# yizhiwang96/Slice3D

Measured on AMD Instinct MI355X. Metric: occupancy query-points/sec (U-Net encode + per-query decode, 256^2 x 12 slices), higher is better.
Workload: dtype f16x3

## Files before the change

include/slice3d_hip.h:

```cpp
#ifndef SLICE3D_HIP_H
#define SLICE3D_HIP_H

#include <stddef.h>
#include <stdint.h>

#ifdef __cplusplus
extern "C" {
#endif

#define S3D_VERSION 118
#define S3D_E_ARG (-1)
#define S3D_E_WORKSPACE (-2)

#define S3D_N_LEVELS 5
#define S3D_D_MODEL 128
#define S3D_N_LAYERS 3
#define S3D_FFN 2048
#define S3D_N_TOKENS_MAX 13

#define S3D_PREC_F32 0
#define S3D_PREC_F16X3 1
#define S3D_PREC_F16 2
#define S3D_PREC_BF16 3

int s3d_version(void);
const char* s3d_last_error(void);


typedef struct {
    const float* w;
    const float* b;
    const float* bn[4];
} S3dConvParams;

typedef struct {
    S3dConvParams enc[13];
    S3dConvParams trans_c;
    S3dConvParams trans_up[4];
    S3dConvParams up_t[4];
    S3dConvParams up_c1[4];
    S3dConvParams up_c2[4];
    S3dConvParams outc;
    const float* emds;
    int n_slices;
} S3dUNetParams;

size_t s3d_unet_packed_bytes(int n_slices);
int s3d_unet_pack(const S3dUNetParams* params_host, void* packed, size_t packed_bytes, void* stream);

typedef struct {
    float* level[S3D_N_LEVELS];
    int n_img;
    int size;
} S3dPyramid;

size_t s3d_unet_workspace_bytes(int batch, int size, int n_slices);
int s3d_unet_encode_fwd(const void* packed, const float* img, const S3dPyramid* out,
                        float* slices_rec, int batch, int size, int n_slices, int prec,
                        void* workspace, size_t workspace_bytes, void* stream);

typedef struct {
    const float* in_proj_w;  const float* in_proj_b;
    const float* out_proj_w; const float* out_proj_b;
// ... 49 lines not shown
    const float* std;
} S3dVggParams;
size_t s3d_vgg_packed_bytes(void);
int s3d_vgg_pack(const S3dVggParams* params_host, void* packed, size_t packed_bytes, void* stream);
size_t s3d_vgg_workspace_bytes(int n_img, int size);
int s3d_vgg_loss_fwd(const void* packed, const float* pred, const float* target, int n_img, int size,
                     float* loss_out, void* workspace, size_t workspace_bytes, void* stream);

typedef struct {
    S3dConvParams conv[13];
} S3dVgg16BnParams;
typedef struct {
    float* level[5];
    int n_img;
    int size;
} S3dGtPyramid;
size_t s3d_gt_encoder_packed_bytes(void);
int s3d_gt_encoder_pack(const S3dVgg16BnParams* params_host, void* packed, size_t packed_bytes, void* stream);
size_t s3d_gt_encoder_workspace_bytes(int n_img, int size);
int s3d_gt_encode_fwd(const void* packed, const float* img_slices, const S3dGtPyramid* out, int n_img, int size,
                      int prec, void* workspace, size_t workspace_bytes, void* stream);

typedef struct {
    const float* pts_w[3];  const float* pts_b[3];
    const float* local_w[2]; const float* local_b[2];
    S3dLayerParams layer[S3D_N_LAYERS];
    const float* fc_out_w; const float* fc_out_b;
} S3dGtHeadParams;
size_t s3d_gt_head_packed_bytes(void);
int s3d_gt_head_pack(const S3dGtHeadParams* params_host, void* packed, size_t packed_bytes, void* stream);
typedef struct {
    float* proj[4];
    const float* fine;
    int n_img;
    int size;
} S3dGtLatent;
int s3d_gt_latent_build(const void* head_packed, const S3dGtPyramid* pyr, const S3dGtLatent* out, int prec,
                        void* stream);
size_t s3d_gt_decode_workspace_bytes(int batch, long n_qry, int n_slices);
int s3d_gt_decode_points_fwd(const void* head_packed, const S3dGtLatent* latent, const float* qry,
                             const float* rot, const float* trans, int flip_yz, float* sdf_out, int batch,
                             long n_qry, int n_slices, int prec, void* workspace, size_t workspace_bytes,
                             void* stream);
int s3d_gt_decode_grid_fwd(const void* head_packed, const S3dGtLatent* latent, const float* trans, int nx,
                           float box, float* logits_out, int n_slices, int prec, void* workspace,
                           size_t workspace_bytes, void* stream);

size_t s3d_conv_packed_bytes(int cout, int cin0, int cin1, int ks);
int s3d_conv_pack(const float* w, const float* bias, int cout, int cin0, int cin1, int ks, void* packed,
                  size_t packed_bytes, void* stream);
int s3d_conv_fwd(const void* packed, const float* x0, const float* x1, const float* residual, float* out, int N,
                 int H, int W, int cout, int cin0, int cin1, int ks, int prec, void* workspace,
                 size_t workspace_bytes, void* stream);
size_t s3d_group_norm_stats_floats(int N, int groups);
int s3d_conv_gn_supported(int cout, int cin0, int cin1, int ks, int prec, int H, int W, int has_workspace);
typedef struct {
    const float* part;
    int nsplit;
    const void* conv_packed;
    int cout, cin0, cin1, ks;
    const float* residual;
    float* out;
} S3dConvPartial;
int s3d_group_norm_table_fwd(const float* x0, int c0, const float* x1, int c1, const float* gamma, const float* beta,
                             const float* film, long film_stride, float* table, float* stats, int N, int HW, int groups,
                             float eps, const S3dConvPartial* x0_partial, void* stream);
int s3d_group_norm_partial_fwd(const S3dConvPartial* x0_partial, const float* gamma, const float* beta, const float* film,
                               long film_stride, float* y, float* stats, int N, int HW, int groups, float eps, int silu,
                               void* stream);
int s3d_conv_gn_fwd(const void* packed, const float* x0, const float* x1, const float* residual, float* out, int N, int H,
                    int W, int cout, int cin0, int cin1, int ks, int prec, const float* table, int silu, void* workspace,
                    size_t workspace_bytes, int* nsplit_out, void* stream);
int s3d_conv_finish_fwd(const S3dConvPartial* partial, int N, int H, int W, void* stream);
int s3d_group_norm_fwd(const float* x, const float* gamma, const float* beta, const float* film, float* y,
                       float* stats, int N, int HW, int C, int groups, float eps, int silu, void* stream);
int s3d_group_norm_film_fwd(const float* x, const float* gamma, const float* beta, const float* film, long film_stride,
                            float* y, float* stats, int N, int HW, int C, int groups, float eps, int silu, void* stream);
int s3d_group_norm2_fwd(const float* x0, int c0, const float* x1, int c1, const float* gamma, const float* beta,
                        const float* film, float* y, float* stats, int N, int HW, int groups, float eps, int silu,
                        void* stream);
int s3d_qkv_attention_fwd(const float* qkv, float* out, int N, int T, int heads, int ch, int prec, void* stream);
size_t s3d_qkv_attention_ws_bytes(int N, int T, int heads, int ch);
int s3d_qkv_attention_ws_fwd(const float* qkv, float* out, int N, int T, int heads, int ch, void* ws, size_t ws_bytes,
                             void* stream);
int s3d_resample2x_fwd(const float* x, float* y, int N, int H, int W, int C, int up, void* stream);
int s3d_small_linear_fwd(const float* x, const float* w, const float* b, float* out, int N, int K, int M,
                         int silu_in, void* stream);
int s3d_timestep_embedding_fwd(const float* t, float* out, int N, int dim, float max_period, void* stream);
int s3d_add_fwd(const float* a, const float* b, float* out, long n, void* stream);
int s3d_nchw_to_nhwc_pad(const float* in, float* out, int n, int c, int h, int w, int cpad, void* stream);
int s3d_add_nchw_fwd(const float* a, const float* b, float* out, int n, int c, int h, int w, void* stream);

int s3d_conv_strided_fwd(const void* packed, const float* x, float* out, int N, int Hin, int Win, int Hout, int Wout, int cout,
                         int cin, int ks, int stride, int pad_origin, int prec, void* stream);
int s3d_wide_attention_fwd(const float* qkv, float* out, int N, int T, int C, int prec, void* stream);
int s3d_image_normalize_fwd(const float* x, const float* mean, const float* std, float* y, int n, int c, int h, int w,
                            void* stream);

typedef int (*s3d_all_reduce_sum_fn)(void* user, float* device_buf, long n_floats, void* stream);
typedef struct {
    s3d_all_reduce_sum_fn all_reduce_sum;
    void* user;
    int world_size;
    float* scratch;
} S3dSyncBn;
typedef struct {
// ... 121 lines not shown
```

slice3d_amd/_lib.py:

```python
import ctypes as C
import os

_HERE = os.path.dirname(os.path.abspath(__file__))
LIB_PATH = os.environ.get("S3D_HIP_LIB") or os.path.join(_HERE, "csrc", "libslice3d_hip.so")

N_LEVELS = 5
N_LAYERS = 3
PREC_F32 = 0
PREC_F16X3 = 1
PREC_F16 = 2
PREC_BF16 = 3
PREC = {"f32": PREC_F32, "f16x3": PREC_F16X3, "f16": PREC_F16, "bf16": PREC_BF16}
PROF_UNET, PROF_LATENT, PROF_SAMPLE, PROF_ATTN, PROF_FFN, PROF_FFN_FINAL, PROF_VGG, PROF_SAMPLE_PYR = range(8)
PROF_NAMES = ("unet_encode", "latent_build", "sample_tokens", "attn_layer", "ffn_layer", "ffn_final", "vgg_loss",
              "sample_pyramid")

c_float_p = C.POINTER(C.c_float)


class S3dConvParams(C.Structure):
    _fields_ = [("w", C.c_void_p), ("b", C.c_void_p), ("bn", C.c_void_p * 4)]


class S3dUNetParams(C.Structure):
# ... 51 lines not shown

class S3dGtHeadParams(C.Structure):
    _fields_ = [("pts_w", C.c_void_p * 3), ("pts_b", C.c_void_p * 3), ("local_w", C.c_void_p * 2),
                ("local_b", C.c_void_p * 2), ("layer", S3dLayerParams * N_LAYERS),
                ("fc_out_w", C.c_void_p), ("fc_out_b", C.c_void_p)]


class S3dGtLatent(C.Structure):
    _fields_ = [("proj", C.c_void_p * 4), ("fine", C.c_void_p), ("n_img", C.c_int), ("size", C.c_int)]


class S3dLatent(C.Structure):
    _fields_ = [("proj", C.c_void_p * 3), ("fine", C.c_void_p * 2), ("n_img", C.c_int),
                ("size", C.c_int)]


_vp, _i, _l, _sz, _f = C.c_void_p, C.c_int, C.c_long, C.c_size_t, C.c_float
SYMBOLS = {
    "s3d_version": (_i, []),
    "s3d_last_error": (C.c_char_p, []),
    "s3d_unet_packed_bytes": (_sz, [_i]),
    "s3d_unet_pack": (_i, [C.POINTER(S3dUNetParams), _vp, _sz, _vp]),
    "s3d_unet_workspace_bytes": (_sz, [_i, _i, _i]),
    "s3d_unet_encode_fwd": (_i, [_vp, _vp, C.POINTER(S3dPyramid), _vp, _i, _i, _i, _i, _vp, _sz, _vp]),
    "s3d_head_packed_bytes": (_sz, []),
    "s3d_head_pack": (_i, [C.POINTER(S3dHeadParams), _vp, _sz, _vp]),
    "s3d_latent_build": (_i, [_vp, C.POINTER(S3dPyramid), C.POINTER(S3dLatent), _i, _vp]),
    "s3d_decode_workspace_bytes": (_sz, [_i, _l, _i]),
    "s3d_decode_workspace_bytes_min": (_sz, [_i, _l, _i]),
    "s3d_decode_set_lanes": (_i, [_i]),
    "s3d_decode_set_last_fused": (_i, [_i]),
    "s3d_decode_set_shared_footprint": (_i, [_i]),
    "s3d_decode_points_fwd": (_i, [_vp, C.POINTER(S3dLatent), _vp, _vp, _vp, _i, _vp, _i, _l, _i, _i,
                                   _vp, _sz, _vp]),
    "s3d_decode_stages_floats": (_sz, [_i, _l, _i]),
    "s3d_decode_points_stages_fwd": (_i, [_vp, C.POINTER(S3dLatent), _vp, _vp, _vp, _i, _vp, _vp, _i, _l, _i, _i,
                                          _vp, _sz, _vp]),
    "s3d_decode_grid_fwd": (_i, [_vp, C.POINTER(S3dLatent), _vp, _i, _f, _vp, _i, _i, _vp, _sz, _vp]),
    "s3d_decode_grid_slab_fwd": (_i, [_vp, C.POINTER(S3dLatent), _vp, _i, _f, _l, _l, _vp, _i, _i, _vp, _sz, _vp]),
    "s3d_gt_encoder_packed_bytes": (_sz, []),
    "s3d_gt_encoder_pack": (_i, [C.POINTER(S3dVgg16BnParams), _vp, _sz, _vp]),
    "s3d_gt_encoder_workspace_bytes": (_sz, [_i, _i]),
    "s3d_gt_encode_fwd": (_i, [_vp, _vp, C.POINTER(S3dGtPyramid), _i, _i, _i, _vp, _sz, _vp]),
    "s3d_gt_head_packed_bytes": (_sz, []),
    "s3d_gt_head_pack": (_i, [C.POINTER(S3dGtHeadParams), _vp, _sz, _vp]),
    "s3d_gt_latent_build": (_i, [_vp, C.POINTER(S3dGtPyramid), C.POINTER(S3dGtLatent), _i, _vp]),
    "s3d_gt_decode_workspace_bytes": (_sz, [_i, _l, _i]),
    "s3d_gt_decode_points_fwd": (_i, [_vp, C.POINTER(S3dGtLatent), _vp, _vp, _vp, _i, _vp, _i, _l, _i, _i,
                                      _vp, _sz, _vp]),
    "s3d_gt_decode_grid_fwd": (_i, [_vp, C.POINTER(S3dGtLatent), _vp, _i, _f, _vp, _i, _i, _vp, _sz, _vp]),
    "s3d_conv_packed_bytes": (_sz, [_i, _i, _i, _i]),
    "s3d_conv_pack": (_i, [_vp, _vp, _i, _i, _i, _i, _vp, _sz, _vp]),
    "s3d_conv_fwd": (_i, [_vp, _vp, _vp, _vp, _vp, _i, _i, _i, _i, _i, _i, _i, _i, _vp, _sz, _vp]),
    "s3d_group_norm_stats_floats": (_sz, [_i, _i]),
    "s3d_group_norm_table_fwd": (_i, [_vp, _i, _vp, _i, _vp, _vp, _vp, C.c_long, _vp, _vp, _i, _i, _i, _f, _vp, _vp]),
    "s3d_group_norm_partial_fwd": (_i, [_vp, _vp, _vp, _vp, C.c_long, _vp, _vp, _i, _i, _i, _f, _i, _vp]),
    "s3d_conv_gn_supported": (_i, [_i, _i, _i, _i, _i, _i, _i, _i]),
    "s3d_conv_gn_fwd": (_i, [_vp, _vp, _vp, _vp, _vp, _i, _i, _i, _i, _i, _i, _i, _i, _vp, _i, _vp, _sz, _vp, _vp]),
    "s3d_conv_finish_fwd": (_i, [_vp, _i, _i, _i, _vp]),
    "s3d_group_norm_fwd": (_i, [_vp, _vp, _vp, _vp, _vp, _vp, _i, _i, _i, _i, _f, _i, _vp]),
    "s3d_group_norm_film_fwd": (_i, [_vp, _vp, _vp, _vp, C.c_long, _vp, _vp, _i, _i, _i, _i, _f, _i, _vp]),
    "s3d_group_norm2_fwd": (_i, [_vp, _i, _vp, _i, _vp, _vp, _vp, _vp, _vp, _i, _i, _i, _f, _i, _vp]),
    "s3d_qkv_attention_fwd": (_i, [_vp, _vp, _i, _i, _i, _i, _i, _vp]),
    "s3d_qkv_attention_ws_bytes": (_sz, [_i, _i, _i, _i]),
    "s3d_qkv_attention_ws_fwd": (_i, [_vp, _vp, _i, _i, _i, _i, _vp, _sz, _vp]),
    "s3d_resample2x_fwd": (_i, [_vp, _vp, _i, _i, _i, _i, _i, _vp]),
    "s3d_small_linear_fwd": (_i, [_vp, _vp, _vp, _vp, _i, _i, _i, _i, _vp]),
    "s3d_timestep_embedding_fwd": (_i, [_vp, _vp, _i, _i, _f, _vp]),
    "s3d_add_fwd": (_i, [_vp, _vp, _vp, _l, _vp]),
    "s3d_nchw_to_nhwc_pad": (_i, [_vp, _vp, _i, _i, _i, _i, _i, _vp]),
    "s3d_add_nchw_fwd": (_i, [_vp, _vp, _vp, _i, _i, _i, _i, _vp]),
    "s3d_conv_strided_fwd": (_i, [_vp, _vp, _vp, _i, _i, _i, _i, _i, _i, _i, _i, _i, _i, _i, _vp]),
    "s3d_wide_attention_fwd": (_i, [_vp, _vp, _i, _i, _i, _i, _vp]),
    "s3d_image_normalize_fwd": (_i, [_vp, _vp, _vp, _vp, _i, _i, _i, _i, _vp]),
    "s3d_vgg_packed_bytes": (_sz, []),
    "s3d_vgg_pack": (_i, [C.POINTER(S3dVggParams), _vp, _sz, _vp]),
    "s3d_vgg_workspace_bytes": (_sz, [_i, _i]),
    "s3d_vgg_loss_fwd": (_i, [_vp, _vp, _vp, _i, _i, _vp, _vp, _sz, _vp]),
    "s3d_train_workspace_bytes": (_sz, [_i, _i, _l, _i]),
    "s3d_train_fwd_bwd": (_i, [C.POINTER(S3dUNetParams), C.POINTER(S3dHeadParams), C.POINTER(S3dVggParams),
                               C.POINTER(S3dUNetParams), C.POINTER(S3dHeadParams), C.POINTER(S3dTrainBatch),
                               _i, _i, _l, _i, _f, C.c_ulonglong, _i, _vp, _vp, _vp, _vp, _sz, _vp]),
    "s3d_train_fwd": (_i, [C.POINTER(S3dUNetParams), C.POINTER(S3dHeadParams), C.POINTER(S3dVggParams),
                           C.POINTER(S3dTrainBatch), _i, _i, _l, _i, _f, C.c_ulonglong, _i, _vp, _vp, _vp, _vp, _sz, _vp]),
    "s3d_train_bwd": (_i, [C.POINTER(S3dUNetParams), C.POINTER(S3dHeadParams), C.POINTER(S3dVggParams),
                           C.POINTER(S3dUNetParams), C.POINTER(S3dHeadParams), C.POINTER(S3dTrainBatch),
                           _i, _i, _l, _i, _f, C.c_ulonglong, _i, _vp, _vp, _f, _f, _vp, _vp, _sz, _vp]),
    "s3d_gt_train_workspace_bytes": (_sz, [_i, _i, _l, _i]),
    "s3d_gt_train_fwd_bwd": (_i, [C.POINTER(S3dVgg16BnParams), C.POINTER(S3dGtHeadParams),
                                  C.POINTER(S3dVgg16BnParams), C.POINTER(S3dGtHeadParams), C.POINTER(S3dTrainBatch),
                                  _i, _i, _l, _i, _f, C.c_ulonglong, _i, _vp, _vp, _vp, _sz, _vp]),
    "s3d_dropout_mask": (_i, [C.c_ulonglong, _i, C.c_ulonglong, _l, _f, _vp, _vp]),
    "s3d_adam_step": (_i, [_vp, _vp, _vp, _vp, _l, _f, _f, _f, _f, _i, _vp]),
    "s3d_adam_step_multi": (_i, [_vp, _vp, _vp, _i, _vp, _vp, _vp, _f, _f, _f, _f, _i, _vp]),
    "s3d_prof_enable": (_i, [_i]),
    "s3d_range_push": (_i, [C.c_char_p]),
    "s3d_range_pop": (_i, []),
    "s3d_prof_read": (_i, [_i, C.POINTER(C.c_double), C.POINTER(C.c_long)]),
    "s3d_project_coord_fwd": (_i, [_vp, _vp, _vp, _i, _l, _vp]),
    "s3d_query_sort_workspace_bytes": (_sz, [_i, _l]),
    "s3d_query_sort": (_i, [_vp, _vp, _vp, _i, _i, _l, _vp, _vp, _sz, _vp]),
    "s3d_sample_pyramid_workspace_bytes": (_sz, [_i, _l]),
    "s3d_sample_pyramid_fwd": (_i, [C.POINTER(S3dPyramid), _vp, _vp, _i, _i, _l, _vp, _sz, _vp]),
    "s3d_sample_planes_fwd": (_i, [_vp, _vp, _vp, _i, _i, _i, _i, _l, _vp]),
    "s3d_mise_dev_workspace_bytes": (_sz, [_i, _i]),
    "s3d_mise_dev_create": (_vp, [_vp, _sz, _i, _i, C.c_double, _vp]),
# ... 81 lines not shown
```

slice3d_amd/csrc/api.hip:

```cpp
#include <dlfcn.h>
#include <stdarg.h>
#include <string.h>

#include <vector>
#include <mutex>

#include <math.h>

#include "conv.h"
#include "decode.h"
#include "train.h"
#include "ldm_ops.h"

static thread_local char g_err[512] = "";

void s3d_set_error(const char* fmt, ...) {
    va_list ap;
    va_start(ap, fmt);
    vsnprintf(g_err, sizeof(g_err), fmt, ap);
    va_end(ap);
}

extern "C" int s3d_version(void) { return S3D_VERSION; }
extern "C" const char* s3d_last_error(void) { return g_err; }
// ... 220 lines not shown
        return S3D_E_WORKSPACE;
    }
    float* base = (float*)packed;
    TRY(pack_encoder(P->enc, base, L.E, st));
    if (hipMemcpyAsync(base + L.enc0_raw, P->enc[0].w, 64 * 27 * sizeof(float), hipMemcpyDeviceToDevice, st) != hipSuccess) {
        s3d_set_error("unet_pack: copy of conv1_1's weight failed");
        return S3D_E_ARG;
    }
    TRY(pack_linear(P->trans_c.w, base + L.trans_c.w, 512, 512, 640, 640, 0, st));
    TRY(pack_linear(P->trans_c.w, base + L.trans_c.w16, 512, 512, 640, 640, 0, st, 1));
    TRY(launch_fold_bn(P->trans_c.b, nullptr, base + L.trans_c.scale, base + L.trans_c.shift, 512, 512, 1, 0, st));
    for (int i = 0; i < 4; ++i) {
        const int C = kUpC[i], Ct = C / 2;
        TRY(pack_linear(P->trans_up[i].w, base + L.trans_up[i].w, Ct, Ct, C, C, 0, st));
        TRY(pack_linear(P->trans_up[i].w, base + L.trans_up[i].w16, Ct, Ct, C, C, 0, st, 1));
        TRY(launch_fold_bn(P->trans_up[i].b, nullptr, base + L.trans_up[i].scale, base + L.trans_up[i].shift, Ct,
                           Ct, 1, 0, st));
        {
            PackArgs a = {};
            a.src = P->up_t[i].w; a.dst = base + L.up_t[i].w; a.kind = S3D_PACK_CONVT;
            a.n_valid = 4 * Ct; a.n_pad = 4 * Ct; a.KU_total = C / 16; a.u_off = 0; a.ku_seg = C / 16;
            a.k_valid = C; a.ct = Ct;
            TRY(launch_pack(a, st));
            a.f16 = 1; a.dst = base + L.up_t[i].w16;
            TRY(launch_pack(a, st));
            TRY(launch_fold_bn(P->up_t[i].b, nullptr, base + L.up_t[i].scale, base + L.up_t[i].shift, Ct, 4 * Ct, 4,
                               0, st));
        }
        TRY(pack_conv3(P->up_c1[i].w, base + L.up_c1[i].w, Ct, Ct, C, 0, Ct, L.up_c1[i].KU, 0, 9, st));
        TRY(pack_conv3(P->up_c1[i].w, base + L.up_c1[i].w, Ct, Ct, C, Ct, Ct, L.up_c1[i].KU, 9 * Ct / 16, 9, st));
        TRY(pack_conv3(P->up_c1[i].w, base + L.up_c1[i].w16, Ct, Ct, C, 0, Ct, L.up_c1[i].KU, 0, 9, st, 1));
        TRY(pack_conv3(P->up_c1[i].w, base + L.up_c1[i].w16, Ct, Ct, C, Ct, Ct, L.up_c1[i].KU, 9 * Ct / 16, 9, st, 1));
        TRY(launch_fold_bn(nullptr, P->up_c1[i].bn, base + L.up_c1[i].scale, base + L.up_c1[i].shift, Ct, Ct, 1, 0,
                           st));
        TRY(pack_conv3(P->up_c2[i].w, base + L.up_c2[i].w, Ct, Ct, Ct, 0, Ct, L.up_c2[i].KU, 0, 9, st));
        TRY(pack_conv3(P->up_c2[i].w, base + L.up_c2[i].w16, Ct, Ct, Ct, 0, Ct, L.up_c2[i].KU, 0, 9, st, 1));
        TRY(launch_fold_bn(nullptr, P->up_c2[i].bn, base + L.up_c2[i].scale, base + L.up_c2[i].shift, Ct, Ct, 1, 0,
                           st));
    }
    TRY(pack_linear(P->outc.w, base + L.outc.w, 3, 16, 32, 32, 0, st));
    TRY(pack_linear(P->outc.w, base + L.outc.w16, 3, 16, 32, 32, 0, st, 1));
    TRY(launch_fold_bn(P->outc.b, nullptr, base + L.outc.scale, base + L.outc.shift, 3, 16, 1, 0, st));
    hipError_t e = hipMemcpyAsync(base + L.emds, P->emds, (size_t)P->n_slices * 128 * sizeof(float),
                                  hipMemcpyDeviceToDevice, st);
    if (e != hipSuccess) {
        s3d_set_error("unet_pack: memcpy failed: %s", hipGetErrorString(e));
        return (int)e;
    }
    return 0;
}

#define S3D_SPLITK_FLOATS ((size_t)4718592)
struct UNetWs {
    size_t in16, a, b, x[5], p[4], proj, up, mid, splitk;
    size_t total;
};
static UNetWs unet_ws(int B, int S, int ns) {
    UNetWs W;
    size_t off = 0;
    auto take = [&](size_t n) {
        size_t o = off;
        off += (n + 63) / 64 * 64;
        return o;
    };
    const size_t px = (size_t)B * S * S;
    W.in16 = take(px * 16);
    W.a = take(px * 64);
    W.b = take(px * 64 / 2);
    const int xc[5] = {64, 128, 256, 512, 512};
    for (int i = 0; i < 5; ++i) W.x[i] = take((px >> (2 * i)) * xc[i]);
    for (int i = 0; i < 4; ++i) W.p[i] = take((px >> (2 * (i + 1))) * xc[i]);
    W.proj = take(px * 32);
    W.up = take(px * ns * 32);
    W.mid = take(px * ns * 32);
    W.splitk = take(S3D_SPLITK_FLOATS);
    W.total = off;
    return W;
}

extern "C" size_t s3d_unet_workspace_bytes(int batch, int size, int n_slices) {
    return unet_ws(batch, size, n_slices).total * sizeof(float);
}

static ConvLaunch conv_desc(const float* base, const PackedConv& pc, int prec, int N, int H, int W, int ks, int act) {
    ConvLaunch c = {};
    c.wpk16 = prec != S3D_PREC_F32 ? (const void*)(base + pc.w16) : nullptr;
    c.single_pass = prec == S3D_PREC_F16;
    c.N = N; c.H = H; c.W = W; c.ks = ks;
    c.CoutPad = pc.cout_pad; c.wpk = base + pc.w; c.KU = pc.KU;
    c.scale = base + pc.scale; c.shift = base + pc.shift;
    c.act = act; c.out_mode = S3D_OUT_NHWC; c.cout_store = pc.cout_pad; c.out_cstride = pc.cout_pad;
    return c;
}
static ConvSrc plain_src(const float* p, int C) { return ConvSrc{p, C, 1, 0, 0}; }

static ConvLaunch proj_desc(const float* w, const void* w16, bool single, int n, int k, const float* x, int N, int H,
                            int W, float* out, const float* shift = nullptr, int act = S3D_ACT_NONE) {
    ConvLaunch c = {};
    c.N = N; c.H = H; c.W = W; c.ks = 1;
    c.CoutPad = n; c.wpk = w; c.KU = k / 16;
    c.wpk16 = w16; c.single_pass = single;
    c.shift = shift; c.act = act;
    c.out_mode = S3D_OUT_NHWC; c.cout_store = n; c.out_cstride = n;
    c.nsrc = 1;
    c.src[0] = plain_src(x, k);
    c.out = out;
    return c;
}

static int encoder_fwd(const float* base, const EncLayout& E, int prec, int N, int S, int first, const float* in,
                       float* const tap[5], float* const pp[2], float* const pool[4], float* splitk, hipStream_t st) {
    const float* cur = in;
    int curC = first ? kEncCout[0] : 16, res = S, tap_i = 0, flip = first;
    for (int i = first; i < 13; ++i) {
        ConvLaunch c = conv_desc(base, E.enc[i], prec, N, res, res, 3, kEncTap[i] ? S3D_ACT_NONE : S3D_ACT_RELU);
        c.nsrc = 1;
        c.src[0] = plain_src(cur, curC);
        c.splitk_ws = splitk; c.splitk_floats = S3D_SPLITK_FLOATS;
        c.out = kEncTap[i] ? tap[tap_i] : pp[flip];
        TRY(launch_conv(c, st));
        cur = c.out;
        curC = kEncCout[i];
        if (!kEncTap[i]) {
            flip ^= 1;
            continue;
// ... 16 lines not shown
    S3D_CHECK_ARG(prec == S3D_PREC_F32 || prec == S3D_PREC_F16X3 || prec == S3D_PREC_F16 || prec == S3D_PREC_BF16,
                  "unet_encode: precision mode %d", prec);
    if (prec == S3D_PREC_BF16) prec = S3D_PREC_F16;
    S3D_CHECK_ARG(packed && img && out && workspace, "unet_encode: null argument");
    S3D_CHECK_ARG(B >= 1 && S >= 16 && S % 16 == 0, "unet_encode: B=%d S=%d (S must be a multiple of 16)", B, S);
    S3D_CHECK_ARG(ns >= 1 && ns <= 12, "unet_encode: n_slices %d", ns);
    S3D_CHECK_ARG(out->n_img == B * ns && out->size == S, "unet_encode: pyramid handle mismatch");
    const UNetLayout L = unet_layout(ns);
    const UNetWs W = unet_ws(B, S, ns);
    if (workspace_bytes < W.total * sizeof(float)) {
        s3d_set_error("unet_encode: workspace %zu < %zu bytes", workspace_bytes, W.total * sizeof(float));
        return S3D_E_WORKSPACE;
    }
    const float* base = (const float*)packed;
    float* ws = (float*)workspace;

    ProfScope prof_(S3D_PROF_UNET, st);
    float* const pp[2] = {ws + W.a, ws + W.b};
    float* const tap[5] = {ws + W.x[0], ws + W.x[1], ws + W.x[2], ws + W.x[3], ws + W.x[4]};
    float* const pool[4] = {ws + W.p[0], ws + W.p[1], ws + W.p[2], ws + W.p[3]};
    TRY(launch_conv3x3_first(img, 3, base + L.enc0_raw, nullptr, pp[0], B, S, S, st, base + L.E.enc[0].scale,
                             base + L.E.enc[0].shift, 1));
    TRY(encoder_fwd(base, L.E, prec, B, S, 1, pp[0], tap, pp, pool, ws + W.splitk, st));
    const int r5 = S / 16;
    {
        ConvLaunch c = conv_desc(base, L.trans_c, prec, B * ns, r5, r5, 1, S3D_ACT_NONE);
        c.nsrc = 2;
        c.src[0] = ConvSrc{ws + W.x[4], 512, ns, 0, 0};
        c.src[1] = ConvSrc{base + L.emds, 128, 1, ns, 1};
        c.out = out->level[0];
        TRY(launch_conv(c, st));
    }
    const float* prev = out->level[0];
    int rp = r5;
    for (int i = 0; i < 4; ++i) {
        const int C = kUpC[i], Ct = C / 2, ro = rp * 2;
        {
            ConvLaunch c = conv_desc(base, L.trans_up[i], prec, B, ro, ro, 1, S3D_ACT_NONE);
            c.nsrc = 1;
            c.src[0] = plain_src(ws + W.x[3 - i], C);
            c.out = ws + W.proj;
            TRY(launch_conv(c, st));
        }
        {
            ConvLaunch c = conv_desc(base, L.up_t[i], prec, B * ns, rp, rp, 1, S3D_ACT_NONE);
            c.nsrc = 1;
            c.src[0] = plain_src(prev, C);
            c.out = ws + W.up;
            c.out_mode = S3D_OUT_CONVT;
            c.cout_store = Ct;
            TRY(launch_conv(c, st));
        }
        {
            ConvLaunch c = conv_desc(base, L.up_c1[i], prec, B * ns, ro, ro, 3, S3D_ACT_RELU);
            c.nsrc = 2;
            c.src[0] = ConvSrc{ws + W.proj, Ct, ns, 0, 0};
            c.src[1] = plain_src(ws + W.up, Ct);
            c.out = ws + W.mid;
            TRY(launch_conv(c, st));
        }
        {
            ConvLaunch c = conv_desc(base, L.up_c2[i], prec, B * ns, ro, ro, 3, S3D_ACT_RELU);
            c.nsrc = 1;
            c.src[0] = plain_src(ws + W.mid, Ct);
            c.out = out->level[i + 1];
            TRY(launch_conv(c, st));
        }
        prev = out->level[i + 1];
        rp = ro;
    }
    if (slices_rec) {
        ConvLaunch c = conv_desc(base, L.outc, prec, B * ns, S, S, 1, S3D_ACT_TANH);
        c.nsrc = 1;
        c.src[0] = plain_src(prev, 32);
        c.out = slices_rec;
        c.out_mode = S3D_OUT_NCHW;
        c.cout_store = 3;
        TRY(launch_conv(c, st));
    }
    return 0;
}

static const int kVggCin[14] = {3, 64, 64, 128, 128, 256, 256, 256, 256, 512, 512, 512, 512, 512};
static const int kVggCout[14] = {64, 64, 128, 128, 256, 256, 256, 256, 512, 512, 512, 512, 512, 512};
static const int kVggPoolAfter[14] = {0, 1, 0, 1, 0, 0, 0, 1, 0, 0, 0, 1, 0, 0};
static const int kVggTap[14] = {0, 1, 0, 2, 0, 3, 0, 0, 0, 4, 0, 0, 0, 5};
static const float kVggW[5] = {1.0f / 2.6f, 1.0f / 4.8f, 1.0f / 3.7f, 1.0f / 5.6f, 10.0f / 1.5f};

struct VggLayout {
    PackedConv conv[14];
    size_t mean, stdv, total;
};
static VggLayout vgg_layout() {
    VggLayout L;
    size_t off = 0;
    auto take = [&](size_t n) {
        size_t o = off;
        off += (n + 3) / 4 * 4;
        return o;
    };
    for (int i = 0; i < 14; ++i) {
        L.conv[i].cout_pad = kVggCout[i];
        L.conv[i].KU = 9 * pad16(kVggCin[i]) / 16;
        L.conv[i].w = take((size_t)kVggCout[i] * L.conv[i].KU * 16);
        L.conv[i].w16 = 0;
        L.conv[i].scale = take(kVggCout[i]);
        L.conv[i].shift = take(kVggCout[i]);
    }
    L.mean = take(4);
    L.stdv = take(4);
// ... 651 lines not shown
```

slice3d_amd/csrc/api_ldm.inc:

```

struct GenConvLayout {
    int cout_pad, KU;
    size_t w, w16, scale, shift, total;
};
static GenConvLayout gen_conv_layout(int cout, int cin0, int cin1, int ks) {
    GenConvLayout L;
    L.cout_pad = pad16(cout);
    const int taps = ks * ks;
    L.KU = taps * (pad16(cin0) + pad16(cin1)) / 16;
    size_t off = 0;
    auto take = [&](size_t n) {
        size_t o = off;
        off += (n + 3) / 4 * 4;
        return o;
    };
    L.w = take((size_t)L.cout_pad * L.KU * 16);
    L.w16 = take((size_t)L.cout_pad * L.KU * 16);
    L.scale = take(L.cout_pad);
    L.shift = take(L.cout_pad);
    L.total = off;
    return L;
}

extern "C" size_t s3d_conv_packed_bytes(int cout, int cin0, int cin1, int ks) {
    return gen_conv_layout(cout, cin0, cin1, ks).total * sizeof(float);
}

extern "C" int s3d_conv_pack(const float* w, const float* bias, int cout, int cin0, int cin1, int ks, void* packed,
                             size_t packed_bytes, void* stream) {
    hipStream_t st = (hipStream_t)stream;
    S3D_CHECK_ARG(w && packed && cout >= 1 && cin0 >= 1 && cin1 >= 0 && (ks == 1 || ks == 3), "conv_pack: bad arguments");
    const GenConvLayout L = gen_conv_layout(cout, cin0, cin1, ks);
    if (packed_bytes < L.total * sizeof(float)) {
        s3d_set_error("conv_pack: packed buffer %zu < %zu bytes", packed_bytes, L.total * sizeof(float));
        return S3D_E_WORKSPACE;
    }
    float* b = (float*)packed;
    const int taps = ks * ks, ct = cin0 + cin1;
    const bool f16 = L.KU % 2 == 0 && cin0 % 32 == 0 && cin1 % 32 == 0;
    TRY(pack_conv3(w, b + L.w, cout, L.cout_pad, ct, 0, cin0, L.KU, 0, taps, st));
    if (f16) TRY(pack_conv3(w, b + L.w16, cout, L.cout_pad, ct, 0, cin0, L.KU, 0, taps, st, 1));
    if (cin1 > 0) {
        TRY(pack_conv3(w, b + L.w, cout, L.cout_pad, ct, cin0, cin1, L.KU, taps * pad16(cin0) / 16, taps, st));
        if (f16) TRY(pack_conv3(w, b + L.w16, cout, L.cout_pad, ct, cin0, cin1, L.KU, taps * pad16(cin0) / 16, taps, st, 1));
    }
    TRY(launch_fold_bn(bias, nullptr, b + L.scale, b + L.shift, cout, L.cout_pad, 1, 0, st));
    return 0;
}

static int conv_fwd_impl(const void* packed, const float* x0, const float* x1, const float* residual, float* out,
                         int N, int H, int W, int cout, int cin0, int cin1, int ks, int prec, void* workspace,
                         size_t workspace_bytes, void* stream, const ConvGn* gn, int* splits_out = nullptr) {
    hipStream_t st = (hipStream_t)stream;
    S3D_CHECK_ARG(packed && x0 && out && N >= 1 && H >= 1 && W >= 1 && (ks == 1 || ks == 3) && cout % 4 == 0,
                  "conv_fwd: bad arguments");
    S3D_CHECK_ARG((cin1 > 0) == (x1 != nullptr), "conv_fwd: x1 / cin1 mismatch");
    const GenConvLayout L = gen_conv_layout(cout, cin0, cin1, ks);
    const float* b = (const float*)packed;
    ConvLaunch c = {};
    c.N = N; c.H = H; c.W = W; c.ks = ks;
    c.CoutPad = L.cout_pad; c.wpk = b + L.w; c.KU = L.KU;
    const bool f16 = L.KU % 2 == 0 && cin0 % 32 == 0 && cin1 % 32 == 0;
    S3D_CHECK_ARG(prec == S3D_PREC_F32 || prec == S3D_PREC_F16X3 || prec == S3D_PREC_F16, "conv_fwd: precision mode %d", prec);
    c.wpk16 = (prec != S3D_PREC_F32 && f16) ? (const void*)(b + L.w16) : nullptr;
    c.single_pass = prec == S3D_PREC_F16 && f16;
    c.scale = nullptr;
    c.shift = b + L.shift; c.act = S3D_ACT_NONE;
    c.out_mode = S3D_OUT_NHWC; c.cout_store = cout; c.out_cstride = cout;
    c.nsrc = cin1 > 0 ? 2 : 1;
    c.src[0] = plain_src(x0, pad16(cin0));
    if (cin1 > 0) c.src[1] = plain_src(x1, pad16(cin1));
    c.out = out; c.residual = residual;
    if (gn) c.gn = *gn;
    c.splits_out = splits_out;
    if (splits_out) *splits_out = 1;
    if (workspace && workspace_bytes >= sizeof(float)) {
        c.splitk_ws = (float*)workspace;
        c.splitk_floats = workspace_bytes / sizeof(float);
    }
    return launch_conv(c, st);
}

extern "C" int s3d_conv_fwd(const void* packed, const float* x0, const float* x1, const float* residual, float* out,
                            int N, int H, int W, int cout, int cin0, int cin1, int ks, int prec, void* workspace,
                            size_t workspace_bytes, void* stream) {
    return conv_fwd_impl(packed, x0, x1, residual, out, N, H, W, cout, cin0, cin1, ks, prec, workspace, workspace_bytes, stream,
                         nullptr);
}
extern "C" int s3d_conv_gn_supported(int cout, int cin0, int cin1, int ks, int prec, int H, int W, int has_workspace) {
    if (ks != 3 || (prec != S3D_PREC_F16X3 && prec != S3D_PREC_F16)) return 0;
    if (cout <= 0 || cin0 <= 0 || cin1 < 0 || cout % 32 || cin0 % 32 || cin1 % 32) return 0;
    if (cin0 + cin1 > S3D_GN_CMAX) return 0;
    if (H > 0 && W > 0 && (W < 16 || H < 8) && !has_workspace) return 0;
    return 1;
}
extern "C" int s3d_conv_gn_fwd(const void* packed, const float* x0, const float* x1, const float* residual, float* out,
                               int N, int H, int W, int cout, int cin0, int cin1, int ks, int prec, const float* table,
                               int silu, void* workspace, size_t workspace_bytes, int* nsplit_out, void* stream) {
    S3D_CHECK_ARG(table, "conv_gn_fwd: null table");
    S3D_CHECK_ARG(s3d_conv_gn_supported(cout, cin0, cin1, ks, prec, H, W, workspace && workspace_bytes >= sizeof(float)),
                  "conv_gn_fwd: needs ks 3, split precision, channel counts that are multiples of 32 (at most %d inputs) and, below "
                  "an 8 x 16 map, a split-K workspace (s3d_conv_gn_supported)", S3D_GN_CMAX);
    const ConvGn gn = {table, silu};
    return conv_fwd_impl(packed, x0, x1, residual, out, N, H, W, cout, cin0, cin1, ks, prec, workspace, workspace_bytes, stream,
                         &gn, nsplit_out);
}
static int partial_to_gn(const S3dConvPartial* p, int N, int HW, GnPartial& g) {
    S3D_CHECK_ARG(p->part && p->out && p->conv_packed && p->nsplit >= 2, "conv partial: bad descriptor");
    const GenConvLayout L = gen_conv_layout(p->cout, p->cin0, p->cin1, p->ks);
    S3D_CHECK_ARG(L.cout_pad == p->cout, "conv partial: cout %d is padded to %d", p->cout, L.cout_pad);
    g.part = p->part; g.nsplit = p->nsplit; g.shift = (const float*)p->conv_packed + L.shift; g.res = p->residual; g.fin = p->out;
    (void)N; (void)HW;
    return 0;
}
extern "C" int s3d_conv_finish_fwd(const S3dConvPartial* p, int N, int H, int W, void* stream) {
    S3D_CHECK_ARG(p, "conv_finish: null descriptor");
    GnPartial g;
    TRY(partial_to_gn(p, N, H * W, g));
    ConvLaunch c = {};
    c.N = N; c.H = H; c.W = W; c.ks = p->ks; c.CoutPad = p->cout;
    c.scale = nullptr; c.shift = g.shift; c.act = S3D_ACT_NONE;
    c.out_mode = S3D_OUT_NHWC; c.cout_store = p->cout; c.out_cstride = p->cout;
    c.out = p->out; c.residual = p->residual;
    c.splitk_ws = const_cast<float*>(p->part);
    return launch_conv_splitk_finish(c, p->nsplit, (hipStream_t)stream);
}
extern "C" size_t s3d_group_norm_stats_floats(int N, int groups) {
    return (size_t)N * groups * S3D_GN_SLICES * 3;
}
extern "C" int s3d_group_norm_table_fwd(const float* x0, int c0, const float* x1, int c1, const float* gamma,
                                        const float* beta, const float* film, long film_stride, float* table, float* stats,
                                        int N, int HW, int groups, float eps, const S3dConvPartial* x0_partial, void* stream) {
    S3D_CHECK_ARG((x0 || x0_partial) && gamma && beta && table && stats && c0 > 0 && c1 >= 0 && (c1 > 0) == (x1 != nullptr),
                  "group_norm_table: bad argument");
    S3D_CHECK_ARG(!film || film_stride >= 2L * (c0 + c1), "group_norm_table: film stride %ld", film_stride);
    GnPartial g;
    if (x0_partial) {
        TRY(partial_to_gn(x0_partial, N, HW, g));
        S3D_CHECK_ARG(x0_partial->cout == c0, "group_norm_table: partial source has %d channels, c0 = %d", x0_partial->cout, c0);
    }
// ... 71 lines not shown
```

slice3d_amd/csrc/conv.h:

```cpp
#pragma once
#include "common.h"
#include "dropout.h"

struct ConvSrc {
    const float* p;
    int C;
    int bdiv, bmod, sbcast;
};

#define S3D_GN_SLICES 64
#define S3D_GN_CMAX 1536
struct ConvGn {
    const float* table;
    int silu;
};

enum { S3D_ACT_NONE = 0, S3D_ACT_RELU = 1, S3D_ACT_TANH = 2 };
enum { S3D_OUT_NHWC = 0, S3D_OUT_CONVT = 1, S3D_OUT_NCHW = 2 };

struct ConvLaunch {
    ConvSrc src[2];
    int nsrc;
    int N, H, W;
    int ks;
    int stride;
    int Hin, Win;
    int pad_origin;
    int CoutPad;
    const float* wpk;
    int KU;
    const void* wpk16;
    int single_pass;
    const float* scale;
    const float* shift;
    int act;
    float* out;
    int out_mode;
    int cout_store;
    int out_cstride;
    const float* residual;
    int out_accumulate;
    int xcd_remap;
    const float* gate;
    float gate_scale;
    unsigned long long drop_base;
    float* splitk_ws;
    size_t splitk_floats;
    DropCfg drop;
    ConvGn gn;
    int* splits_out;
};

int launch_conv(const ConvLaunch& a, hipStream_t stream);
int launch_conv_splitk_finish(const ConvLaunch& a, int nsplit, hipStream_t stream);

enum { S3D_PACK_LINEAR = 0, S3D_PACK_CONV = 1, S3D_PACK_CONVT = 2, S3D_PACK_CONV_DGRAD = 3,
       S3D_PACK_CONVT_DGRAD = 4, S3D_PACK_LINEAR_T = 5 };
struct PackArgs {
    const float* src;
    float* dst;
    int kind;
    int n_valid, n_pad;
    int KU_total, u_off, ku_seg;
    int ld, k_valid;
    int taps, cseg, cseg_valid, cin_tot, cin_begin;
    int ct;
    int f16;
    int chunk_ku;
};
int launch_pack(const PackArgs& a, hipStream_t stream);
class PackBatchScope {
public:
    PackBatchScope();
    ~PackBatchScope();
    int flush(hipStream_t stream);
    PackBatchScope(const PackBatchScope&) = delete;
    PackBatchScope& operator=(const PackBatchScope&) = delete;
private:
    void* prev_;
    void* q_;
};
class PackBatchSuspend {
public:
    PackBatchSuspend();
    ~PackBatchSuspend();
private:
    void* saved_;
};
int launch_fold_bn(const float* bias, const float* const bn[4], float* scale, float* shift, int c_valid,
                   int c_pad, int rep, int bias_before_bn, hipStream_t stream);

int launch_bn_relu_pool(const float* in, const float* scale, const float* shift, float* out, int n, int h,
// ... 12 lines not shown
```

slice3d_amd/csrc/conv.hip:

```cpp
#include <stdlib.h>
#include "conv.h"
#include <vector>

template <int MT, int NT>
__device__ __forceinline__ void conv_epilogue(const ConvLaunch& a, f32x4 (&acc)[MT][NT], const int (&pn)[MT],
                                              const int (&py)[MT], const int (&px)[MT], const bool (&pv)[MT],
                                              int jt0, int g) {
    const bool convt32 = a.out_mode == S3D_OUT_CONVT && a.cout_store % 32 == 0;
    if (NT % 2 == 0 && (a.out_mode == S3D_OUT_NHWC || convt32)) {
        const int m = threadIdx.x & 15;
        const bool lo = m < 8;
#pragma unroll
        for (int np = 0; np < NT / 2; ++np) {
            const int co = (jt0 + 2 * np) * 16 + 16 * (m >> 3) + 4 * g;
            const f32x4 sc = a.scale ? ld4(a.scale + co) : f32x4{1.f, 1.f, 1.f, 1.f};
            const f32x4 sh = a.shift ? ld4(a.shift + co) : zero4();
            const int ct = a.cout_store, cq = convt32 ? co / ct : 0, ccol = convt32 ? co - cq * ct : co;
            const bool col_ok = convt32 ? cq < 4 : co < a.cout_store;
#pragma unroll
            for (int mt = 0; mt < MT; ++mt) {
                f32x4 val[2];
                s3d_full_line_pair(acc[mt][2 * np], acc[mt][2 * np + 1], m, val[0], val[1]);
                const long ob = convt32 ? ((long)(pn[mt] * 2 * a.H + 2 * py[mt] + (cq >> 1)) * (2 * a.W) + 2 * px[mt] + (cq & 1)) * ct
                                        : ((long)(pn[mt] * a.H + py[mt]) * a.W + px[mt]) * a.out_cstride;
                const unsigned ob_lo = s3d_row_ror8_u32((unsigned)ob), ob_hi = s3d_row_ror8_u32((unsigned)((unsigned long long)ob >> 32));
                const bool pvp = s3d_row_ror8_u32(pv[mt] ? 1u : 0u) != 0u;
                const long obp = (long)(((unsigned long long)ob_hi << 32) | ob_lo);
#pragma unroll
                for (int k = 0; k < 2; ++k) {
                    const bool own = (k == 0) == lo;
                    if (!(own ? pv[mt] : pvp) || !col_ok) continue;
                    const long oi = (own ? ob : obp) + ccol;
                    f32x4 v = val[k] * sc + sh;
                    if (a.act == S3D_ACT_RELU) {
#pragma unroll
                        for (int i = 0; i < 4; ++i) v[i] = fmaxf(v[i], 0.f);
                    } else if (a.act == S3D_ACT_TANH) {
#pragma unroll
                        for (int i = 0; i < 4; ++i) v[i] = tanhf(v[i]);
                    }
                    if (a.drop.p > 0.f) {
#pragma unroll
                        for (int i = 0; i < 4; ++i) v[i] *= s3d_drop(a.drop, a.drop_base + (unsigned long long)(oi + i));
                    }
                    if (a.gate) {
                        const f32x4 gt = ld4(a.gate + oi);
#pragma unroll
                        for (int i = 0; i < 4; ++i) v[i] = gt[i] > 0.f ? v[i] * a.gate_scale : 0.f;
                    }
                    if (a.residual) v += ld4(a.residual + oi);
                    if (a.out_accumulate) v += ld4(a.out + oi);
                    __builtin_nontemporal_store(v, reinterpret_cast<f32x4*>(a.out + oi));
                }
                __builtin_amdgcn_sched_barrier(0);
            }
        }
        return;
    }
#pragma unroll
    for (int nt = 0; nt < NT; ++nt) {
        const int co = (jt0 + nt) * 16 + 4 * g;
        const f32x4 sc = a.scale ? ld4(a.scale + co) : f32x4{1.f, 1.f, 1.f, 1.f};
        const f32x4 sh = a.shift ? ld4(a.shift + co) : zero4();
#pragma unroll
        for (int mt = 0; mt < MT; ++mt) {
            if (!pv[mt]) continue;
            f32x4 v = acc[mt][nt] * sc + sh;
            if (a.act == S3D_ACT_RELU) {
#pragma unroll
                for (int i = 0; i < 4; ++i) v[i] = fmaxf(v[i], 0.f);
            } else if (a.act == S3D_ACT_TANH) {
#pragma unroll
                for (int i = 0; i < 4; ++i) v[i] = tanhf(v[i]);
            }
            if (a.out_mode == S3D_OUT_NHWC) {
                if (co < a.cout_store) {
                    const long oi = ((long)(pn[mt] * a.H + py[mt]) * a.W + px[mt]) * a.out_cstride + co;
                    if (a.drop.p > 0.f) {
#pragma unroll
                        for (int i = 0; i < 4; ++i) v[i] *= s3d_drop(a.drop, a.drop_base + (unsigned long long)(oi + i));
                    }
                    if (a.gate) {
                        const f32x4 gt = ld4(a.gate + oi);
#pragma unroll
                        for (int i = 0; i < 4; ++i) v[i] = gt[i] > 0.f ? v[i] * a.gate_scale : 0.f;
                    }
                    if (a.residual) v += ld4(a.residual + oi);
                    if (a.out_accumulate) v += ld4(a.out + oi);
                    __builtin_nontemporal_store(v, reinterpret_cast<f32x4*>(a.out + oi));
                }
            } else if (a.out_mode == S3D_OUT_CONVT) {
                const int ct = a.cout_store;
                const int q = co / ct, c = co - q * ct;
                if (q < 4) {
                    const int oy = 2 * py[mt] + (q >> 1), ox = 2 * px[mt] + (q & 1);
                    float* o = a.out + ((long)(pn[mt] * 2 * a.H + oy) * (2 * a.W) + ox) * ct + c;
                    st4(o, v);
                }
            } else {
#pragma unroll
                for (int i = 0; i < 4; ++i)
                    if (co + i < a.cout_store)
                        a.out[((long)(pn[mt] * a.cout_store + co + i) * a.H + py[mt]) * a.W + px[mt]] = v[i];
            }
        }
    }
}

__device__ __forceinline__ void conv_block_tile(const ConvLaunch& a, int n_co_blk, int& blk_co, long& blk_px) {
    const long L = blockIdx.x;
    if (!a.xcd_remap || n_co_blk == 1) {
        blk_co = (int)(L % n_co_blk);
        blk_px = L / n_co_blk;
        return;
    }
    const long n_px = gridDim.x / n_co_blk, full = n_px & ~7L, lim = full * n_co_blk;
    if (L < lim) {
        const long k = L >> 3;
        blk_co = (int)(k % n_co_blk);
        blk_px = (k / n_co_blk) * 8 + (L & 7);
// ... 1063 lines not shown
    } else {
        if (one) hipLaunchKernelGGL((conv3x3_lds_f16x3_kernel<2, 4, 1, 1>), grid, dim3(256), 0, stream, a, tiles_x, tiles_y, cps);
        else hipLaunchKernelGGL((conv3x3_lds_f16x3_kernel<2, 4, 1, 2>), grid, dim3(256), 0, stream, a, tiles_x, tiles_y, cps);
    }
    S3D_LAUNCH_CHECK();
    if (a.splits_out) {
        *a.splits_out = splits;
        if (splits > 1) return 0;
    }
    if (splits > 1) return launch_conv_splitk_finish(a, splits, stream);
    return 0;
}

template <int MT, int NT, int WM, int WN>
static int launch_cfg(const ConvLaunch& a, hipStream_t stream) {
    constexpr int PIX_WG = WM * MT * 16, CO_WG = WN * NT * 16;
    const long P = (long)a.N * a.H * a.W;
    const long nblk = ((P + PIX_WG - 1) / PIX_WG) * (a.CoutPad / CO_WG);
    S3D_CHECK_ARG(nblk > 0 && nblk < (1L << 31), "conv grid out of range (%ld)", nblk);
    dim3 grid((unsigned)nblk), block(WM * WN * 64);
    bool f16 = a.wpk16 != nullptr && (a.KU % 2 == 0);
    for (int s = 0; s < a.nsrc; ++s) f16 = f16 && (a.src[s].C % 32 == 0);
    if (f16) {
        if (a.ks == 3)
            hipLaunchKernelGGL((conv_igemm_f16x3_kernel<MT, NT, WM, WN, 3>), grid, block, 0, stream, a);
        else if (a.ks == 2)
            hipLaunchKernelGGL((conv_igemm_f16x3_kernel<MT, NT, WM, WN, 2>), grid, block, 0, stream, a);
        else
            hipLaunchKernelGGL((conv_igemm_f16x3_kernel<MT, NT, WM, WN, 1>), grid, block, 0, stream, a);
        S3D_LAUNCH_CHECK();
        return 0;
    }
    if (a.ks == 3)
        hipLaunchKernelGGL((conv_igemm_kernel<MT, NT, WM, WN, 3>), grid, block, 0, stream, a);
    else if (a.ks == 2)
        hipLaunchKernelGGL((conv_igemm_kernel<MT, NT, WM, WN, 2>), grid, block, 0, stream, a);
    else
        hipLaunchKernelGGL((conv_igemm_kernel<MT, NT, WM, WN, 1>), grid, block, 0, stream, a);
    S3D_LAUNCH_CHECK();
    return 0;
}

int launch_conv(const ConvLaunch& a_in, hipStream_t stream) {
    ConvLaunch a = a_in;
    a.xcd_remap = 1;
    S3D_CHECK_ARG(a.ks >= 1 && a.ks <= 3, "conv: ks must be 1, 2 or 3");
    S3D_CHECK_ARG(!a.pad_origin || (a.ks == 3 && a.stride > 1 && a.out_mode == S3D_OUT_NHWC),
                  "conv: pad_origin is served for strided 3x3 convolutions only");
    S3D_CHECK_ARG(a.CoutPad % 16 == 0 && a.CoutPad > 0, "conv: CoutPad %d", a.CoutPad);
    for (int s = 0; s < a.nsrc; ++s)
        S3D_CHECK_ARG(a.src[s].C % 16 == 0 && a.src[s].bdiv >= 1, "conv: bad source %d", s);
    S3D_CHECK_ARG(a.out_mode != S3D_OUT_CONVT || (a.drop.p <= 0.f && !a.gate && !a.residual && !a.out_accumulate),
                  "conv: ConvTranspose output takes no dropout / gate / residual / accumulate");
    if (conv3x3_lds_eligible(a)) return launch_conv3x3_lds(a, stream);
    S3D_CHECK_ARG(!a.gn.table, "conv: a fused GroupNorm needs the LDS-staged 3x3 kernel (ks 3, stride 1, channel counts multiples of 32)");
    if (conv1x1_small_eligible(a)) {
        bool served = false;
        const int rc = launch_conv1x1_small(a, stream, served);
        if (rc || served) return rc;
    }
    if (lin_stream_eligible(a)) return launch_lin_stream(a, stream);
    if (lin_rows_eligible(a)) return launch_lin_rows(a, stream);
    const long P = (long)a.N * a.H * a.W;
    const long want = 512;
    auto nblk = [&](int pix, int co) { return ((P + pix - 1) / pix) * (a.CoutPad / co); };
    if (a.CoutPad % 128 == 0) {
        if (nblk(128, 128) >= want) return launch_cfg<4, 4, 2, 2>(a, stream);
        if (nblk(64, 128) >= want) return launch_cfg<2, 4, 2, 2>(a, stream);
        if (a.CoutPad % 128 == 0 && nblk(32, 128) >= want / 2) return launch_cfg<1, 4, 2, 2>(a, stream);
        return launch_cfg<1, 1, 2, 2>(a, stream);
    }
    if (a.CoutPad % 64 == 0) {
        if (nblk(256, 64) >= want) return launch_cfg<4, 4, 4, 1>(a, stream);
        if (nblk(64, 64) >= want / 2) return launch_cfg<2, 2, 2, 2>(a, stream);
        return launch_cfg<1, 1, 2, 2>(a, stream);
    }
    if (a.CoutPad % 32 == 0) {
        if (nblk(256, 32) >= want) return launch_cfg<4, 2, 4, 1>(a, stream);
        return launch_cfg<1, 1, 2, 2>(a, stream);
    }
    if (nblk(256, 16) >= want) return launch_cfg<4, 1, 4, 1>(a, stream);
    return launch_cfg<1, 1, 4, 1>(a, stream);
}

__device__ __forceinline__ void pack_frag_body(const PackArgs& a) {
    const long total = (long)(a.n_pad / 16) * a.ku_seg * 256;
    for (long idx = (long)blockIdx.x * blockDim.x + threadIdx.x; idx < total;
         idx += (long)gridDim.x * blockDim.x) {
        int e, lane, ul, j, k;
        if (!a.f16) {
            e = idx & 3; lane = (idx >> 2) & 63;
            const long fu = idx >> 8;
            ul = (int)(fu % a.ku_seg); j = (int)(fu / a.ku_seg);
            k = 16 * ul + 4 * (lane >> 4) + e;
        } else {
            const int t = idx & 7;
            lane = (idx >> 3) & 63;
            const long fu = idx >> 9;
            const int u32 = (int)(fu % (a.ku_seg / 2));
            j = (int)(fu / (a.ku_seg / 2));
            k = 32 * u32 + 8 * (lane >> 4) + t;
            ul = u32; e = t;
        }
        const int n = 16 * j + (lane & 15);
        float v = 0.f;
        if (n < a.n_valid) {
            if (a.kind == S3D_PACK_LINEAR) {
                if (k < a.k_valid) v = a.src[(long)n * a.ld + k];
            } else if (a.kind == S3D_PACK_CONV) {
                const int tap = k / a.cseg, c = k - tap * a.cseg;
                if (c < a.cseg_valid) v = a.src[((long)n * a.cin_tot + a.cin_begin + c) * a.taps + tap];
            } else if (a.kind == S3D_PACK_CONVT) {
                const int q = n / a.ct, co = n - q * a.ct;
// ... 371 lines not shown
```

Before: 11.66 million.

## Split shared skip half of up-conv into a once-per-batch pre-activation addend

The U-Net up-block conv concatenated a projection input that is broadcast across the ns slices (bdiv=ns) with a per-slice upsampled input, so the projection half of the 3x3 conv was recomputed for every slice. That half is now computed once per batch item into a new workspace buffer, and the per-slice conv only processes the upsampled channels (weight pointer offset past the first Ct inputs) and adds the precomputed result before ReLU through a new 'pre' epilogue addend. This cuts the FLOPs of that conv roughly in half, at the cost of an extra launch, an extra buffer, and extra epilogue loads. A public conv_pre_fwd entry point is also added.

```diff
diff --git a/include/slice3d_hip.h b/include/slice3d_hip.h
--- a/include/slice3d_hip.h
+++ b/include/slice3d_hip.h
@@ -8,7 +8,7 @@
 extern "C" {
 #endif
 
-#define S3D_VERSION 118
+#define S3D_VERSION 119
 #define S3D_E_ARG (-1)
 #define S3D_E_WORKSPACE (-2)
 
@@ -164,6 +164,9 @@
 int s3d_conv_fwd(const void* packed, const float* x0, const float* x1, const float* residual, float* out, int N,
                  int H, int W, int cout, int cin0, int cin1, int ks, int prec, void* workspace,
                  size_t workspace_bytes, void* stream);
+int s3d_conv_pre_fwd(const void* packed, const float* x0, const float* x1, int x0_bdiv, const float* pre, int pre_bdiv, int act,
+                     float* out, int N, int H, int W, int cout, int cin0, int cin1, int ks, int prec, void* workspace,
+                     size_t workspace_bytes, void* stream);
 size_t s3d_group_norm_stats_floats(int N, int groups);
 int s3d_conv_gn_supported(int cout, int cin0, int cin1, int ks, int prec, int H, int W, int has_workspace);
 typedef struct {
diff --git a/slice3d_amd/_lib.py b/slice3d_amd/_lib.py
--- a/slice3d_amd/_lib.py
+++ b/slice3d_amd/_lib.py
@@ -127,6 +127,7 @@
     "s3d_conv_packed_bytes": (_sz, [_i, _i, _i, _i]),
     "s3d_conv_pack": (_i, [_vp, _vp, _i, _i, _i, _i, _vp, _sz, _vp]),
     "s3d_conv_fwd": (_i, [_vp, _vp, _vp, _vp, _vp, _i, _i, _i, _i, _i, _i, _i, _i, _vp, _sz, _vp]),
+    "s3d_conv_pre_fwd": (_i, [_vp, _vp, _vp, _i, _vp, _i, _i, _vp, _i, _i, _i, _i, _i, _i, _i, _i, _vp, _sz, _vp]),
     "s3d_group_norm_stats_floats": (_sz, [_i, _i]),
     "s3d_group_norm_table_fwd": (_i, [_vp, _i, _vp, _i, _vp, _vp, _vp, C.c_long, _vp, _vp, _i, _i, _i, _f, _vp, _vp]),
     "s3d_group_norm_partial_fwd": (_i, [_vp, _vp, _vp, _vp, C.c_long, _vp, _vp, _i, _i, _i, _f, _i, _vp]),
diff --git a/slice3d_amd/csrc/api.hip b/slice3d_amd/csrc/api.hip
--- a/slice3d_amd/csrc/api.hip
+++ b/slice3d_amd/csrc/api.hip
@@ -296,7 +296,7 @@
 
 #define S3D_SPLITK_FLOATS ((size_t)4718592)
 struct UNetWs {
-    size_t in16, a, b, x[5], p[4], proj, up, mid, splitk;
+    size_t in16, a, b, x[5], p[4], proj, skip, up, mid, splitk;
     size_t total;
 };
 static UNetWs unet_ws(int B, int S, int ns) {
@@ -315,6 +315,7 @@
     for (int i = 0; i < 5; ++i) W.x[i] = take((px >> (2 * i)) * xc[i]);
     for (int i = 0; i < 4; ++i) W.p[i] = take((px >> (2 * (i + 1))) * xc[i]);
     W.proj = take(px * 32);
+    W.skip = take(px * 32);
     W.up = take(px * ns * 32);
     W.mid = take(px * ns * 32);
     W.splitk = take(S3D_SPLITK_FLOATS);
@@ -437,10 +438,20 @@
             TRY(launch_conv(c, st));
         }
         {
+            ConvLaunch c = conv_desc(base, L.up_c1[i], prec, B, ro, ro, 3, S3D_ACT_NONE);
+            c.nsrc = 1;
+            c.src[0] = plain_src(ws + W.proj, Ct);
+            c.splitk_ws = ws + W.splitk; c.splitk_floats = S3D_SPLITK_FLOATS;
+            c.out = ws + W.skip;
+            TRY(launch_conv(c, st));
+        }
+        {
             ConvLaunch c = conv_desc(base, L.up_c1[i], prec, B * ns, ro, ro, 3, S3D_ACT_RELU);
-            c.nsrc = 2;
-            c.src[0] = ConvSrc{ws + W.proj, Ct, ns, 0, 0};
-            c.src[1] = plain_src(ws + W.up, Ct);
+            c.wpk += (size_t)(9 * Ct / 16) * 256;
+            if (c.wpk16) c.wpk16 = (const _Float16*)c.wpk16 + (size_t)(9 * Ct / 32) * 1024;
+            c.nsrc = 1;
+            c.src[0] = plain_src(ws + W.up, Ct);
+            c.pre = ws + W.skip; c.pre_bdiv = ns;
             c.out = ws + W.mid;
             TRY(launch_conv(c, st));
         }
diff --git a/slice3d_amd/csrc/api_ldm.inc b/slice3d_amd/csrc/api_ldm.inc
--- a/slice3d_amd/csrc/api_ldm.inc
+++ b/slice3d_amd/csrc/api_ldm.inc
@@ -50,7 +50,8 @@
 
 static int conv_fwd_impl(const void* packed, const float* x0, const float* x1, const float* residual, float* out,
                          int N, int H, int W, int cout, int cin0, int cin1, int ks, int prec, void* workspace,
-                         size_t workspace_bytes, void* stream, const ConvGn* gn, int* splits_out = nullptr) {
+                         size_t workspace_bytes, void* stream, const ConvGn* gn, int* splits_out = nullptr, int x0_bdiv = 1,
+                         const float* pre = nullptr, int pre_bdiv = 1, int act = S3D_ACT_NONE) {
     hipStream_t st = (hipStream_t)stream;
     S3D_CHECK_ARG(packed && x0 && out && N >= 1 && H >= 1 && W >= 1 && (ks == 1 || ks == 3) && cout % 4 == 0,
                   "conv_fwd: bad arguments");
@@ -68,9 +69,10 @@
     c.shift = b + L.shift; c.act = S3D_ACT_NONE;
     c.out_mode = S3D_OUT_NHWC; c.cout_store = cout; c.out_cstride = cout;
     c.nsrc = cin1 > 0 ? 2 : 1;
-    c.src[0] = plain_src(x0, pad16(cin0));
+    c.src[0] = ConvSrc{x0, pad16(cin0), x0_bdiv, 0, 0};
     if (cin1 > 0) c.src[1] = plain_src(x1, pad16(cin1));
     c.out = out; c.residual = residual;
+    c.act = act; c.pre = pre; c.pre_bdiv = pre_bdiv;
     if (gn) c.gn = *gn;
     c.splits_out = splits_out;
     if (splits_out) *splits_out = 1;
@@ -86,6 +88,14 @@
                             size_t workspace_bytes, void* stream) {
     return conv_fwd_impl(packed, x0, x1, residual, out, N, H, W, cout, cin0, cin1, ks, prec, workspace, workspace_bytes, stream,
                          nullptr);
+}
+extern "C" int s3d_conv_pre_fwd(const void* packed, const float* x0, const float* x1, int x0_bdiv, const float* pre, int pre_bdiv,
+                                int act, float* out, int N, int H, int W, int cout, int cin0, int cin1, int ks, int prec,
+                                void* workspace, size_t workspace_bytes, void* stream) {
+    S3D_CHECK_ARG(pre && pre_bdiv >= 1 && x0_bdiv >= 1, "conv_pre_fwd: pre %p, pre_bdiv %d, x0_bdiv %d", (const void*)pre, pre_bdiv, x0_bdiv);
+    S3D_CHECK_ARG(act == S3D_ACT_NONE || act == S3D_ACT_RELU, "conv_pre_fwd: activation %d (0 none, 1 ReLU)", act);
+    return conv_fwd_impl(packed, x0, x1, nullptr, out, N, H, W, cout, cin0, cin1, ks, prec, workspace, workspace_bytes, stream,
+                         nullptr, nullptr, x0_bdiv, pre, pre_bdiv, act);
 }
 extern "C" int s3d_conv_gn_supported(int cout, int cin0, int cin1, int ks, int prec, int H, int W, int has_workspace) {
     if (ks != 3 || (prec != S3D_PREC_F16X3 && prec != S3D_PREC_F16)) return 0;
diff --git a/slice3d_amd/csrc/conv.h b/slice3d_amd/csrc/conv.h
--- a/slice3d_amd/csrc/conv.h
+++ b/slice3d_amd/csrc/conv.h
@@ -38,6 +38,8 @@
     int out_mode;
     int cout_store;
     int out_cstride;
+    const float* pre;
+    int pre_bdiv;
     const float* residual;
     int out_accumulate;
     int xcd_remap;
diff --git a/slice3d_amd/csrc/conv.hip b/slice3d_amd/csrc/conv.hip
--- a/slice3d_amd/csrc/conv.hip
+++ b/slice3d_amd/csrc/conv.hip
@@ -26,12 +26,14 @@
                 const unsigned ob_lo = s3d_row_ror8_u32((unsigned)ob), ob_hi = s3d_row_ror8_u32((unsigned)((unsigned long long)ob >> 32));
                 const bool pvp = s3d_row_ror8_u32(pv[mt] ? 1u : 0u) != 0u;
                 const long obp = (long)(((unsigned long long)ob_hi << 32) | ob_lo);
+                const int pd = a.pre ? pn[mt] - pn[mt] / a.pre_bdiv : 0;
+                const int pdp = a.pre ? (int)s3d_row_ror8_u32((unsigned)pd) : 0;
 #pragma unroll
                 for (int k = 0; k < 2; ++k) {
                     const bool own = (k == 0) == lo;
                     if (!(own ? pv[mt] : pvp) || !col_ok) continue;
                     const long oi = (own ? ob : obp) + ccol;
-                    f32x4 v = val[k] * sc + sh;
+                    f32x4 v = val[k] * sc + (a.pre ? ld4(a.pre + (oi - (long)(own ? pd : pdp) * a.H * a.W * a.out_cstride)) : sh);
                     if (a.act == S3D_ACT_RELU) {
 #pragma unroll
                         for (int i = 0; i < 4; ++i) v[i] = fmaxf(v[i], 0.f);
@@ -66,6 +68,8 @@
         for (int mt = 0; mt < MT; ++mt) {
             if (!pv[mt]) continue;
             f32x4 v = acc[mt][nt] * sc + sh;
+            if (a.pre && co < a.cout_store)
+                v = acc[mt][nt] * sc + ld4(a.pre + ((long)((pn[mt] / a.pre_bdiv) * a.H + py[mt]) * a.W + px[mt]) * a.out_cstride + co);
             if (a.act == S3D_ACT_RELU) {
 #pragma unroll
                 for (int i = 0; i < 4; ++i) v[i] = fmaxf(v[i], 0.f);
@@ -1235,6 +1239,8 @@
         S3D_CHECK_ARG(a.src[s].C % 16 == 0 && a.src[s].bdiv >= 1, "conv: bad source %d", s);
     S3D_CHECK_ARG(a.out_mode != S3D_OUT_CONVT || (a.drop.p <= 0.f && !a.gate && !a.residual && !a.out_accumulate),
                   "conv: ConvTranspose output takes no dropout / gate / residual / accumulate");
+    S3D_CHECK_ARG(!a.pre || (a.out_mode == S3D_OUT_NHWC && a.pre_bdiv >= 1), "conv: a pre-activation addend needs NHWC output and pre_bdiv >= 1");
+    S3D_CHECK_ARG(!a.pre || !a.splits_out, "conv: a pre-activation addend cannot be combined with a deferred split-K finish");
     if (conv3x3_lds_eligible(a)) return launch_conv3x3_lds(a, stream);
     S3D_CHECK_ARG(!a.gn.table, "conv: a fused GroupNorm needs the LDS-staged 3x3 kernel (ks 3, stride 1, channel counts multiples of 32)");
     if (conv1x1_small_eligible(a)) {
@@ -1242,6 +1248,7 @@
         const int rc = launch_conv1x1_small(a, stream, served);
         if (rc || served) return rc;
     }
+    S3D_CHECK_ARG(!a.pre || !lin_stream_eligible(a), "conv: the streaming row-linear kernel takes no pre-activation addend");
     if (lin_stream_eligible(a)) return launch_lin_stream(a, stream);
     if (lin_rows_eligible(a)) return launch_lin_rows(a, stream);
     const long P = (long)a.N * a.H * a.W;
```

Result: no change. 11.76 million, median of 6 (+0.8%).
